# leoelm/Bayesian_inference_for_NN

Measured on NVIDIA B200. Metric: posterior_grad_evals_per_s, higher is better.
Workload: dtype f32 (tensor-core products on two int8 fixed-point slices per operand, kind::i8, exact int32 accumulate; f32 everywhere else)

## Files before the change

bayesian_inference_for_nn_b200/csrc/tc_fused.cuh:

```cuda
#pragma once
#include "tc_layer2.cuh"

namespace pyb {

constexpr int TF_THREADS = 384;
template <int CP> struct TfCfg {
  static constexpr int STAGES = 5;
  static constexpr int W2_BYTES = 2 * 256 * CP * 4;
  static constexpr int ZX_BYTES = 2 * CP * 128 * 4;
  static constexpr int SMEM = STAGES * TP_STAGE_BYTES + 1024  + 1024  + 2048  +
                              128  + W2_BYTES + ZX_BYTES;
  static constexpr int SMEM_I8 = SMEM + 4096;
};
__device__ __forceinline__ void tc_ld_16x256b_x4_raw(uint32_t taddr, uint32_t* r) {
  asm volatile(
      "tcgen05.ld.sync.aligned.16x256b.x4.b32 "
      "{%0, %1, %2, %3, %4, %5, %6, %7, %8, %9, %10, %11, %12, %13, %14, %15}, [%16];"
      : "=r"(r[0]), "=r"(r[1]), "=r"(r[2]), "=r"(r[3]), "=r"(r[4]), "=r"(r[5]), "=r"(r[6]), "=r"(r[7]), "=r"(r[8]),
        "=r"(r[9]), "=r"(r[10]), "=r"(r[11]), "=r"(r[12]), "=r"(r[13]), "=r"(r[14]), "=r"(r[15])
      : "r"(taddr)
      : "memory");
}
__device__ __forceinline__ void tc_mma_i8_pair(uint32_t tmem_d, uint64_t adesc, uint64_t bdesc, uint32_t idesc,
                                               uint32_t accumulate) {
  asm volatile(
      "{\n"
      ".reg .pred p;\n"
      "setp.ne.b32 p, %4, 0;\n"
      "tcgen05.mma.cta_group::2.kind::i8 [%0], %1, %2, %3, p;\n"
      "}\n" ::"r"(tmem_d),
      "l"(adesc), "l"(bdesc), "r"(idesc), "r"(accumulate)
      : "memory");
}
__device__ __forceinline__ void slice4_i8(const float* d, float zq, uint32_t& hw, uint32_t& lw) {
  constexpr float M = 12582912.0f;
  uint32_t hb[4], lb[4];
#pragma unroll
  for (int r = 0; r < 4; ++r) {
    const float t = fmaf(d[r], zq, M);
    const float h = t - M;
    const float e = fmaf(d[r], zq, -h);
    const float u = fmaf(e, 254.0f, M);
    hb[r] = __float_as_uint(t);
    lb[r] = __float_as_uint(u);
  }
  hw = __byte_perm(__byte_perm(hb[0], hb[1], 0x0040), __byte_perm(hb[2], hb[3], 0x0040), 0x5410);
  lw = __byte_perm(__byte_perm(lb[0], lb[1], 0x0040), __byte_perm(lb[2], lb[3], 0x0040), 0x5410);
}

__device__ __forceinline__ void tc_ld_16x256b_x4(uint32_t taddr, float* v) {
  uint32_t r[16];
  asm volatile(
      "tcgen05.ld.sync.aligned.16x256b.x4.b32 "
      "{%0, %1, %2, %3, %4, %5, %6, %7, %8, %9, %10, %11, %12, %13, %14, %15}, [%16];"
      : "=r"(r[0]), "=r"(r[1]), "=r"(r[2]), "=r"(r[3]), "=r"(r[4]), "=r"(r[5]), "=r"(r[6]), "=r"(r[7]), "=r"(r[8]),
        "=r"(r[9]), "=r"(r[10]), "=r"(r[11]), "=r"(r[12]), "=r"(r[13]), "=r"(r[14]), "=r"(r[15])
      : "r"(taddr)
      : "memory");
#pragma unroll
  for (int i = 0; i < 16; ++i) v[i] = __uint_as_float(r[i]);
}
template <int CP>
__device__ __forceinline__ int w2_slot(int h, int c) {
  return ((((h >> 3) * 2 + (h & 1)) * (CP / 4) + (c >> 2)) * 4 + ((h >> 1) & 3)) * 4 + (c & 3);
}
__device__ __forceinline__ void split_pair(float x0, float x1, uint32_t& hw, uint32_t& lw) {
  const __nv_bfloat162 hp = __floats2bfloat162_rn(x0, x1);
  hw = *reinterpret_cast<const uint32_t*>(&hp);
  const __nv_bfloat162 lp = __floats2bfloat162_rn(x0 - __uint_as_float(hw << 16), x1 - __uint_as_float(hw & 0xffff0000u));
  lw = *reinterpret_cast<const uint32_t*>(&lp);
}

template <int CP, bool FWD, int I8 = 0>
__global__ void __cluster_dims__(2, 1, 1) __launch_bounds__(TF_THREADS, 1)
tc_g1_layer2_fused(const __grid_constant__ CUtensorMap tmA_hi, const __grid_constant__ CUtensorMap tmA_lo,
                   const __grid_constant__ CUtensorMap tmB_hi, const __grid_constant__ CUtensorMap tmB_lo,
                   const TcGemmParams p, const Layer2Params l2) {
  constexpr int STAGES = TfCfg<CP>::STAGES;
  extern __shared__ uint8_t smem_raw[];
  uint8_t* smem = smem_raw + ((1024u - (smem_u32(smem_raw) & 1023u)) & 1023u);
  uint8_t* stage_base = smem;
  uint64_t* bars = (uint64_t*)(smem + STAGES * TP_STAGE_BYTES);
  uint64_t* full_bar = bars;
  uint64_t* empty_bar = bars + STAGES;
  uint64_t* tmem_full = bars + 2 * STAGES;
  uint64_t* tmem_empty = bars + 2 * STAGES + 2;
  uint32_t* tmem_ptr = (uint32_t*)(bars + 2 * STAGES + 4);
  float* bias_s = (float*)(smem + STAGES * TP_STAGE_BYTES + 1024);
  float* b2_s = bias_s + 512;
  float* W2_s = b2_s + 32;
  float* zx_s = W2_s + 2 * 256 * CP;
  float* cw_s = zx_s + 2 * CP * 128;
  float* zq_s = cw_s + 512;

  const int warp = __shfl_sync(0xffffffffu, (int)(threadIdx.x >> 5), 0), lane = threadIdx.x & 31;
  const uint32_t rank = cluster_ctarank();
  const int cluster_id = blockIdx.x >> 1, n_clusters = gridDim.x >> 1;
  constexpr int KSTAGE = I8 ? 64 : TC_BK;
  const int nk = (p.K + KSTAGE - 1) / KSTAGE;
  const int H = p.H;
  const int half_rows = H >> 1;
  const uint32_t cta_bytes = 2 * TC_A_TILE_BYTES + 2 * (uint32_t)half_rows * TC_BK * 2;

  if (warp == 8 && lane == 0) {
    asm volatile("prefetch.tensormap [%0];" ::"l"(&tmA_hi) : "memory");
    asm volatile("prefetch.tensormap [%0];" ::"l"(&tmA_lo) : "memory");
    asm volatile("prefetch.tensormap [%0];" ::"l"(&tmB_hi) : "memory");
    asm volatile("prefetch.tensormap [%0];" ::"l"(&tmB_lo) : "memory");
  }
  if (warp == 9 && lane == 0) {
    for (int s = 0; s < STAGES; ++s) { mbar_init(&full_bar[s], 1); mbar_init(&empty_bar[s], 1); }
    mbar_init(&tmem_full[0], 1); mbar_init(&tmem_full[1], 1);
    mbar_init(&tmem_empty[0], 16); mbar_init(&tmem_empty[1], 16);
    asm volatile("fence.mbarrier_init.release.cluster;" ::: "memory");
  }
  if (warp == 10) {
    asm volatile("tcgen05.alloc.cta_group::2.sync.aligned.shared::cta.b32 [%0], %1;" ::"r"(smem_u32(tmem_ptr)), "r"(512)
                 : "memory");
    asm volatile("tcgen05.relinquish_alloc_permit.cta_group::2.sync.aligned;" ::: "memory");
  }
  tc_fence_before();
  __syncthreads();
  cluster_sync_all();
  tc_fence_after();
  const uint32_t tmem_base = *tmem_ptr;

  if (warp >= 8) {
   asm volatile("setmaxnreg.dec.sync.aligned.u32 40;");
   if (warp == 8) {
    if (lane == 0) {
      int stage = 0;
      uint32_t phase = 0;
      for (int item = cluster_id; item < p.total_items; item += n_clusters) {
        int b, mp, split;
        tc_decode(p, item, b, mp, split);
        const int arow = p.a_row0 + (mp * 2 + (int)rank) * 128;
        const int brow = b * H + (int)rank * half_rows;
        for (int kc = 0; kc < nk; ++kc) {
          (I8 ? mbar_wait_sleep(&empty_bar[stage], phase ^ 1) : mbar_wait(&empty_bar[stage], phase ^ 1));
          uint8_t* st = stage_base + stage * TP_STAGE_BYTES;
          if (rank == 0) mbar_expect_tx(&full_bar[stage], 2 * cta_bytes);
          const int k0 = kc * KSTAGE;
          tma_load_2d_pair(st, &tmA_hi, &full_bar[stage], k0, arow);
          tma_load_2d_pair(st + TC_A_TILE_BYTES, &tmA_lo, &full_bar[stage], k0, arow);
          tma_load_2d_pair(st + 2 * TC_A_TILE_BYTES, &tmB_hi, &full_bar[stage], k0, brow);
          tma_load_2d_pair(st + 2 * TC_A_TILE_BYTES + 8192, &tmB_lo, &full_bar[stage], k0, brow);
          if (++stage == STAGES) { stage = 0; phase ^= 1; }
        }
      }
    }
  } else if (warp == 9) {
    if (rank == 0 && lane == 0) {
      const uint32_t idesc = (I8 ? (2u << 4) : (1u << 4)) | (1u << 7) | (1u << 10) | ((uint32_t)(H >> 3) << 17) | ((256u >> 4) << 24);
      int stage = 0, it = 0;
      uint32_t phase = 0;
      const int k_tail = p.K - (nk - 1) * KSTAGE;
      for (int item = cluster_id; item < p.total_items; item += n_clusters, ++it) {
        const int acc = I8 ? 0 : (it & 1);
        const uint32_t acc_phase = I8 ? (uint32_t)(it & 1) : (uint32_t)((it >> 1) & 1);
        (I8 ? mbar_wait_sleep(&tmem_empty[acc], acc_phase ^ 1) : mbar_wait(&tmem_empty[acc], acc_phase ^ 1));
        tc_fence_after();
        const uint32_t d = tmem_base + (uint32_t)acc * 256;
        for (int kc = 0; kc < nk; ++kc) {
          (I8 ? mbar_wait_sleep(&full_bar[stage], phase) : mbar_wait(&full_bar[stage], phase));
          tc_fence_after();
          const uint32_t st = smem_u32(stage_base + stage * TP_STAGE_BYTES);
          const int nks = (kc == nk - 1 && k_tail <= KSTAGE / 2) ? 1 : 2;
          for (int ks = 0; ks < nks; ++ks) {
            const uint32_t koff = ks * 32;
            const uint64_t ah = make_smem_desc_sw64(st + koff);
            const uint64_t al = make_smem_desc_sw64(st + TC_A_TILE_BYTES + koff);
            const uint64_t bh = make_smem_desc_sw64(st + 2 * TC_A_TILE_BYTES + koff);
            const uint64_t bl = make_smem_desc_sw64(st + 2 * TC_A_TILE_BYTES + 8192 + koff);
            const uint32_t accum = (kc != 0) || (ks != 0);
            if (I8) {
              tc_mma_i8_pair(d, ah, bh, idesc, accum);
              tc_mma_i8_pair(d + 256, ah, bl, idesc, accum);
              tc_mma_i8_pair(d + 256, al, bh, idesc, 1);
            } else {
              tc_mma_bf16_pair(d, ah, bh, idesc, accum);
              tc_mma_bf16_pair(d, al, bh, idesc, 1);
              tc_mma_bf16_pair(d, ah, bl, idesc, 1);
            }
          }
          tc_commit_pair(&empty_bar[stage]);
          if (++stage == STAGES) { stage = 0; phase ^= 1; }
        }
        tc_commit_pair(&tmem_full[acc]);
      }
    }
   }
  } else {
    asm volatile("setmaxnreg.inc.sync.aligned.u32 232;");
    const int half = warp >> 2;
    const int quad = warp & 3;
    const int g = lane >> 2, t = lane & 3;
    const int eall = threadIdx.x;
    const uint32_t lane_addr = (uint32_t)(quad * 32) << 16;
    const int Hh = H >> 1;
    const int C = l2.C;
    const float invN = l2.scale / (float)l2.N;
    const int r_own = 2 * (t & 1) + (t >> 1);
    const int row_own = quad * 32 + g + 8 * r_own;
    const int pos0 = quad * 32 + 4 * g;
    const int hbase = half * Hh + 2 * t;
    uint16_t* z2_hi = reinterpret_cast<uint16_t*>(l2.z2_hi);
    uint16_t* z2_lo = reinterpret_cast<uint16_t*>(l2.z2_lo);
    for (int i = eall; i < 2 * 256 * CP; i += 256) W2_s[i] = 0.f;
    if (eall < 32) b2_s[eall] = 0.f;
    asm volatile("bar.sync 1, 256;" ::: "memory");
    auto fetch_consts = [&](int item, int buf) {
      int b, mp, split;
      tc_decode(p, item, b, mp, split);
      const float* th = l2.theta + (int64_t)b * l2.P;
      if (eall < H) {
        const int h = eall;
        const float* src = th + l2.w2_off + (int64_t)h * C;
        const uint32_t dst = smem_u32(W2_s + buf * 256 * CP + w2_slot<CP>(h, 0));
#pragma unroll
        for (int c = 0; c < CP; ++c)
          if (c < C)
            asm volatile("cp.async.ca.shared.global [%0], [%1], 4;" ::"r"(dst + (uint32_t)(((c >> 2) * 16 + (c & 3)) * 4)),
                         "l"(src + c) : "memory");
        asm volatile("cp.async.ca.shared.global [%0], [%1], 4;" ::"r"(smem_u32(bias_s + buf * 256 + h)),
                     "l"(p.bias + (int64_t)b * p.bias_stride + h) : "memory");
      }
      if (eall < C)
        asm volatile("cp.async.ca.shared.global [%0], [%1], 4;" ::"r"(smem_u32(b2_s + buf * 16 + eall)),
                     "l"(th + l2.b2_off + eall) : "memory");
      if (I8 && eall < H) {
        asm volatile("cp.async.ca.shared.global [%0], [%1], 4;" ::"r"(smem_u32(cw_s + buf * 256 + eall)),
                     "l"(l2.cw + (int64_t)b * H + eall) : "memory");
        if (I8 == 2 && !FWD)
          asm volatile("cp.async.ca.shared.global [%0], [%1], 4;" ::"r"(smem_u32(zq_s + buf * 256 + eall)),
                       "l"(l2.zq + (int64_t)b * H + eall) : "memory");
      }
    };
    if (cluster_id < p.total_items) fetch_consts(cluster_id, 0);
    int it = 0;
    for (int item = cluster_id; item < p.total_items; item += n_clusters, ++it) {
      int b, mp, split;
      tc_decode(p, item, b, mp, split);
      const int mt = mp * 2 + (int)rank;
      const int cbuf = it & 1;
      const int acc = I8 ? 0 : cbuf;
      const uint32_t acc_phase = I8 ? (uint32_t)(it & 1) : (uint32_t)((it >> 1) & 1);
      float* bs = bias_s + cbuf * 256;
      float* b2b = b2_s + cbuf * 16;
      float* W2b = W2_s + cbuf * 256 * CP;
      float sxr[4] = {0.f, 0.f, 0.f, 0.f};
      if (I8) {
#pragma unroll
        for (int r = 0; r < 4; ++r) {
          const int rg = mt * 128 + quad * 32 + g + 8 * r;
          sxr[r] = rg < p.M_valid ? __ldg(l2.sx + rg) : 0.f;
        }
      }
      asm volatile("cp.async.wait_all;" ::: "memory");
      asm volatile("bar.sync 1, 256;" ::: "memory");
      (I8 ? mbar_wait_sleep(&tmem_full[acc], acc_phase) : mbar_wait(&tmem_full[acc], acc_phase));
      tc_fence_after();
      const int64_t blk_w = (((((int64_t)b * p.out_tiles + mt) * H) + hbase) * 128 + pos0) >> 2;
      uint2* pa_hi = reinterpret_cast<uint2*>(p.out_hi) + blk_w;
      uint2* pa_lo = reinterpret_cast<uint2*>(p.out_lo) + blk_w;
      uint2* pz_hi = reinterpret_cast<uint2*>(l2.zt_hi) + blk_w;
      uint2* pz_lo = reinterpret_cast<uint2*>(l2.zt_lo) + blk_w;
      const float4* w4b = reinterpret_cast<const float4*>(W2b) + (((half * Hh) >> 3) * 2 * (CP / 4)) * 4 + t;
      const float* bsb = bs + hbase;
      const float* cwb = cw_s + cbuf * 256 + hbase;
      const float* zqb = zq_s + cbuf * 256 + hbase;
      uint32_t* pzi_hi = nullptr; uint32_t* pzi_lo = nullptr;
      if (I8 == 2 && !FWD) {
        const int64_t blk_b = ((((int64_t)b * p.out_tiles + mt) * H) + hbase) * 128 + pos0;
        pzi_hi = reinterpret_cast<uint32_t*>(l2.zi_hi + blk_b);
        pzi_lo = reinterpret_cast<uint32_t*>(l2.zi_lo + blk_b);
      }
      float2 z[4][CP / 2];
#pragma unroll
      for (int r = 0; r < 4; ++r)
#pragma unroll
        for (int c = 0; c < CP / 2; ++c) z[r][c] = make_float2(0.f, 0.f);
      uint32_t mask[4] = {0u, 0u, 0u, 0u};
#pragma unroll
      for (int ch = 0; ch < 4; ++ch) {
        if (ch * 32 < Hh) {
          const uint32_t col = (uint32_t)(acc * 256 + half * Hh + ch * 32);
          float v[32];
          if (I8) {
#pragma unroll
            for (int hf = 0; hf < 2; ++hf) {
              uint32_t rh[16], rc[16];
              tc_ld_16x256b_x4_raw(tmem_base + lane_addr + ((uint32_t)(16 * hf) << 16) + col, rh);
              tc_ld_16x256b_x4_raw(tmem_base + lane_addr + ((uint32_t)(16 * hf) << 16) + 256u + col, rc);
              asm volatile("tcgen05.wait::ld.sync.aligned;" ::: "memory");
#pragma unroll
              for (int j = 0; j < 16; ++j)
                v[16 * hf + j] = fmaf((float)(int)rc[j], 1.0f / 254.0f, (float)(int)rh[j]);
            }
          } else {
            tc_ld_16x256b_x4(tmem_base + lane_addr + col, v);
            tc_ld_16x256b_x4(tmem_base + lane_addr + (16u << 16) + col, v + 16);
            asm volatile("tcgen05.wait::ld.sync.aligned;" ::: "memory");
          }
          uint32_t m = 0u;
#pragma unroll
          for (int kb = 0; kb < 4; ++kb) {
            const float2 bb = *reinterpret_cast<const float2*>(bsb + ch * 32 + 8 * kb);
            float2 cc = make_float2(0.f, 0.f);
            if (I8) cc = *reinterpret_cast<const float2*>(cwb + ch * 32 + 8 * kb);
            float a[4][2];
#pragma unroll
            for (int r = 0; r < 4; ++r) {
              const float* vv = v + (r >> 1) * 16 + kb * 4 + (r & 1) * 2;
              if (I8) {
                a[r][0] = fmaxf(fmaf(vv[0], sxr[r] * cc.x, bb.x), 0.f);
                a[r][1] = fmaxf(fmaf(vv[1], sxr[r] * cc.y, bb.y), 0.f);
              } else {
                a[r][0] = fmaxf(vv[0] + bb.x, 0.f);
                a[r][1] = fmaxf(vv[1] + bb.y, 0.f);
              }
              if (!FWD) {
                m |= (a[r][0] > 0.f ? 1u : 0u) << (kb * 8 + r * 2);
                m |= (a[r][1] > 0.f ? 1u : 0u) << (kb * 8 + r * 2 + 1);
              }
            }
#pragma unroll
            for (int i = 0; i < 2; ++i) {
              const float4* w4 = w4b + (((ch * 4 + kb) * 2 + i) * (CP / 4)) * 4;
#pragma unroll
              for (int c4 = 0; c4 < CP / 4; ++c4) {
                const float4 w = w4[c4 * 4];
                const float2 w01 = make_float2(w.x, w.y), w23 = make_float2(w.z, w.w);
#pragma unroll
                for (int r = 0; r < 4; ++r) {
                  const float2 aa = make_float2(a[r][i], a[r][i]);
                  z[r][2 * c4] = __ffma2_rn(aa, w01, z[r][2 * c4]);
                  z[r][2 * c4 + 1] = __ffma2_rn(aa, w23, z[r][2 * c4 + 1]);
                }
              }
              if (!FWD) {
                uint32_t hw0, lw0, hw1, lw1;
                split_pair(a[0][i], a[1][i], hw0, lw0);
                split_pair(a[2][i], a[3][i], hw1, lw1);
                const int w_off = (ch * 32 + 8 * kb + i) * 32;
                __stcs(pa_hi + w_off, make_uint2(hw0, hw1));
                __stcs(pa_lo + w_off, make_uint2(lw0, lw1));
              }
            }
          }
          mask[ch] = m;
        }
      }
      tc_fence_before();
      __syncwarp();
      if (lane == 0) mbar_arrive_leader_relaxed(&tmem_empty[acc]);
      if (item + n_clusters < p.total_items) fetch_consts(item + n_clusters, cbuf ^ 1);
      float zo[CP];
      {
        const bool b0 = t & 1, b1 = t & 2;
#pragma unroll
        for (int c = 0; c < CP; ++c) {
          const float z0 = (c & 1) ? z[0][c >> 1].y : z[0][c >> 1].x, z1 = (c & 1) ? z[1][c >> 1].y : z[1][c >> 1].x;
          const float z2v = (c & 1) ? z[2][c >> 1].y : z[2][c >> 1].x, z3 = (c & 1) ? z[3][c >> 1].y : z[3][c >> 1].x;
          float k0 = b0 ? z2v : z0, k1 = b0 ? z3 : z1;
          const float g0 = __shfl_xor_sync(0xffffffffu, b0 ? z0 : z2v, 1);
          const float g1 = __shfl_xor_sync(0xffffffffu, b0 ? z1 : z3, 1);
          k0 = b0 ? g0 + k0 : k0 + g0;
          k1 = b0 ? g1 + k1 : k1 + g1;
          const float kk = b1 ? k1 : k0;
          const float gg = __shfl_xor_sync(0xffffffffu, b1 ? k0 : k1, 2);
          zo[c] = b1 ? gg + kk : kk + gg;
        }
      }
#pragma unroll
      for (int c = 0; c < CP; ++c) zx_s[(half * CP + c) * 128 + row_own] = zo[c];
      asm volatile("bar.sync 2, 256;" ::: "memory");
      float zf[CP], dz[CP];
#pragma unroll
      for (int c = 0; c < CP; ++c) zf[c] = (b2b[c] + zx_s[c * 128 + row_own]) + zx_s[(CP + c) * 128 + row_own];
      const int row_g = mt * 128 + row_own;
      if (FWD) {
        if (half == 0 && row_g < p.M_valid) {
          float* o = l2.fwd_out + ((int64_t)b * l2.N + row_g) * C;
          if (l2.out_act == PYB_ACT_SOFTMAX) {
            float mx = -INFINITY;
#pragma unroll
            for (int c = 0; c < CP; ++c) if (c < C) mx = fmaxf(mx, zf[c]);
            float se = 0.f;
#pragma unroll
            for (int c = 0; c < CP; ++c) if (c < C) se += expf(zf[c] - mx);
            const float inv = 1.0f / se;
#pragma unroll
            for (int c = 0; c < CP; ++c) if (c < C) o[c] = expf(zf[c] - mx) * inv;
          } else {
#pragma unroll
            for (int c = 0; c < CP; ++c) if (c < C) o[c] = act_apply(zf[c], l2.out_act);
          }
        }
        continue;
      }
      float loss_r = 0.f;
      l2_loss_dz<CP>(l2, row_g, row_g < p.M_valid, zf, dz, loss_r, invN);
      if (half == 0) {
        const int64_t blk2 = (((int64_t)b * p.out_tiles + mt) * L2_CMAX) * 128 + pos0 + r_own;
#pragma unroll
        for (int c = 0; c < CP; ++c) {
          __nv_bfloat16 hb, lb;
          split_bf16(dz[c], hb, lb);
          z2_hi[blk2 + c * 128] = __bfloat16_as_ushort(hb);
          z2_lo[blk2 + c * 128] = __bfloat16_as_ushort(lb);
        }
        const int64_t grp = (int64_t)b * l2.n_groups + mt * 4 + quad;
        float mine = 0.f;
#pragma unroll
        for (int c = 0; c < CP; ++c) {
          const float sm = warp_sum(dz[c]);
          if (lane == c) mine = sm;
        }
        if (lane < CP) l2.b2_partial[grp * L2_CMAX + lane] = mine;
        const float ls = warp_sum(loss_r);
        if (lane == 0) l2.loss_partial[grp] = (double)ls;
      }
      float2 dzp[4][CP / 2];
#pragma unroll
      for (int r = 0; r < 4; ++r) {
        const int src = (lane & ~3) | ((r >> 1) | ((r & 1) << 1));
#pragma unroll
        for (int c = 0; c < CP / 2; ++c) {
          dzp[r][c].x = __shfl_sync(0xffffffffu, dz[2 * c], src);
          dzp[r][c].y = __shfl_sync(0xffffffffu, dz[2 * c + 1], src);
        }
      }
#pragma unroll
      for (int ch = 0; ch < 4; ++ch) {
        if (ch * 32 < Hh) {
          const uint32_t m = mask[ch];
#pragma unroll
          for (int kb = 0; kb < 4; ++kb) {
#pragma unroll
            for (int i = 0; i < 2; ++i) {
              const float4* w4 = w4b + (((ch * 4 + kb) * 2 + i) * (CP / 4)) * 4;
              float2 s[4];
#pragma unroll
              for (int r = 0; r < 4; ++r) s[r] = make_float2(0.f, 0.f);
#pragma unroll
              for (int c4 = 0; c4 < CP / 4; ++c4) {
                const float4 w = w4[c4 * 4];
                const float2 w01 = make_float2(w.x, w.y), w23 = make_float2(w.z, w.w);
#pragma unroll
                for (int r = 0; r < 4; ++r) {
                  s[r] = __ffma2_rn(dzp[r][2 * c4], w01, s[r]);
                  s[r] = __ffma2_rn(dzp[r][2 * c4 + 1], w23, s[r]);
                }
              }
              float d[4];
#pragma unroll
              for (int r = 0; r < 4; ++r) d[r] = ((m >> (kb * 8 + r * 2 + i)) & 1u) ? s[r].x + s[r].y : 0.f;
              const int w_off = (ch * 32 + 8 * kb + i) * 32;
              if (I8 == 2) {
                uint32_t hw, lw;
                slice4_i8(d, zqb[ch * 32 + 8 * kb + i], hw, lw);
                __stcs(pzi_hi + w_off, hw);
                __stcs(pzi_lo + w_off, lw);
              } else {
                uint32_t hw0, lw0, hw1, lw1;
                split_pair(d[0], d[1], hw0, lw0);
                split_pair(d[2], d[3], hw1, lw1);
                __stcs(pz_hi + w_off, make_uint2(hw0, hw1));
                __stcs(pz_lo + w_off, make_uint2(lw0, lw1));
              }
            }
          }
        }
      }
    }
  }
  tc_fence_before();
  __syncthreads();
  cluster_sync_all();
  if (warp == 10) {
    tc_fence_after();
    asm volatile("tcgen05.dealloc.cta_group::2.sync.aligned.b32 %0, %1;" ::"r"(tmem_base), "r"(512) : "memory");
  }
}

}
```

bayesian_inference_for_nn_b200/csrc/tc_path.cu:

```cuda
#include <cstdlib>
#include <cstring>
#include "tc_fused_mma.cuh"
#include <algorithm>

namespace pyb {

typedef CUresult (*PFN_encodeTiled)(CUtensorMap*, CUtensorMapDataType, cuuint32_t, void*, const cuuint64_t*,
                                    const cuuint64_t*, const cuuint32_t*, const cuuint32_t*, CUtensorMapInterleave,
                                    CUtensorMapSwizzle, CUtensorMapL2promotion, CUtensorMapFloatOOBfill);
static PFN_encodeTiled get_encode() {
  static PFN_encodeTiled fn = nullptr;
  if (!fn) {
    void* f = nullptr;
    cudaDriverEntryPointQueryResult q;
    PYB_CUDA(cudaGetDriverEntryPoint("cuTensorMapEncodeTiled", &f, cudaEnableDefault, &q));
    PYB_REQUIRE(f != nullptr && q == cudaDriverEntryPointSuccess, PYB_ERR_CUDA, "cuTensorMapEncodeTiled unavailable");
    fn = (PFN_encodeTiled)f;
  }
  return fn;
}
static CUtensorMap make_map_blocked(const void* base, int64_t blocks, int rows_per_block, int box_rows) {
  CUtensorMap m;
  cuuint64_t dims[3] = {128, (cuuint64_t)rows_per_block, (cuuint64_t)blocks};
  cuuint64_t strides[2] = {256, (cuuint64_t)rows_per_block * 256};
// ... 124 lines not shown
  tc_gemm_bf16x3<EPI, ACT><<<grid, TC_THREADS, TC_SMEM_BYTES, h->stream>>>(a_hi, a_lo, b_hi, b_lo, p);
}
template <int EPI, int ACT>
static void launch_pair_inst(pyb_handle* h, int grid, const CUtensorMap& a_hi, const CUtensorMap& a_lo,
                             const CUtensorMap& b_hi, const CUtensorMap& b_lo, const TcGemmParams& p) {
  PYB_CUDA(cudaFuncSetAttribute(tc_gemm_pair_bf16x3<EPI, ACT>, cudaFuncAttributeMaxDynamicSharedMemorySize, TP_SMEM_BYTES));
  tc_gemm_pair_bf16x3<EPI, ACT><<<grid, TP_THREADS, TP_SMEM_BYTES, h->stream>>>(a_hi, a_lo, b_hi, b_lo, p);
}
static bool pair_ok(const pyb_handle* h, const TcGemmParams& p) {
  if (!h->opt_tc_pair || p.b_blocked || p.H < 32 || p.n_mtiles < 2) return false;
  if (p.n_btiles > 0) return p.a_blocked && p.n_mtiles == 2 && (p.H % 16) == 0;
  if ((p.H % 32) != 0) return false;
  return !p.a_blocked && p.a_batch_rows == 0;
}
static void launch_gemm_tc(pyb_handle* h, const CUtensorMap& a_hi, const CUtensorMap& a_lo,
                           const CUtensorMap& b_hi, const CUtensorMap& b_lo, TcGemmParams p, double flops,
                           const CUtensorMap* bp_hi = nullptr, const CUtensorMap* bp_lo = nullptr) {
  if (p.k_splits <= 1) { p.k_splits = 1; p.chunks_per_split = (p.K + TC_BK - 1) / TC_BK; p.split_stride = 0; }
  p.vec_store = p.epi == EPI_STORE && ((uintptr_t)p.out % 16 == 0) && (p.out_stride % 4 == 0) && (p.out_ld % 4 == 0) &&
                (p.split_stride % 4 == 0);
  int grid = std::min(p.total_items, h->sm_count);
  prof_begin(h);
  if (bp_hi && bp_lo && pair_ok(h, p) && p.n_btiles > 1 && p.epi == EPI_STORE && p.transpose_out && h->opt_tc_dual &&
      p.H <= 256 && (p.H / 2) * TC_BK * 2 <= 8192) {
    p.total_items = p.n_batch * p.k_splits * ((p.n_btiles + 1) / 2);
    grid = std::min(2 * p.total_items, (h->sm_count / 2) * 2);
    PYB_CUDA(cudaFuncSetAttribute(tc_gemm_pair_dual_bf16x3, cudaFuncAttributeMaxDynamicSharedMemorySize, TD_SMEM_BYTES));
    tc_gemm_pair_dual_bf16x3<<<grid, TP_THREADS, TD_SMEM_BYTES, h->stream>>>(a_hi, a_lo, *bp_hi, *bp_lo, p);
    prof_end(h, flops);
    count_launch(h);
    return;
  }
  if (bp_hi && bp_lo && pair_ok(h, p)) {
    grid = std::min(2 * p.total_items, (h->sm_count / 2) * 2);
    if (p.epi == EPI_STORE) launch_pair_inst<EPI_STORE, 0>(h, grid, a_hi, a_lo, *bp_hi, *bp_lo, p);
    else if (p.act == PYB_ACT_RELU) launch_pair_inst<EPI_BIAS_ACT_T_SPLIT, PYB_ACT_RELU>(h, grid, a_hi, a_lo, *bp_hi, *bp_lo, p);
    else if (p.act == PYB_ACT_TANH) launch_pair_inst<EPI_BIAS_ACT_T_SPLIT, PYB_ACT_TANH>(h, grid, a_hi, a_lo, *bp_hi, *bp_lo, p);
    else if (p.act == PYB_ACT_SIGMOID) launch_pair_inst<EPI_BIAS_ACT_T_SPLIT, PYB_ACT_SIGMOID>(h, grid, a_hi, a_lo, *bp_hi, *bp_lo, p);
    else launch_pair_inst<EPI_BIAS_ACT_T_SPLIT, PYB_ACT_LINEAR>(h, grid, a_hi, a_lo, *bp_hi, *bp_lo, p);
    prof_end(h, flops);
    count_launch(h);
    return;
  }
  if (p.epi == EPI_STORE) launch_gemm_inst<EPI_STORE, 0>(h, grid, a_hi, a_lo, b_hi, b_lo, p);
  else if (p.act == PYB_ACT_RELU) launch_gemm_inst<EPI_BIAS_ACT_T_SPLIT, PYB_ACT_RELU>(h, grid, a_hi, a_lo, b_hi, b_lo, p);
  else if (p.act == PYB_ACT_TANH) launch_gemm_inst<EPI_BIAS_ACT_T_SPLIT, PYB_ACT_TANH>(h, grid, a_hi, a_lo, b_hi, b_lo, p);
  else if (p.act == PYB_ACT_SIGMOID) launch_gemm_inst<EPI_BIAS_ACT_T_SPLIT, PYB_ACT_SIGMOID>(h, grid, a_hi, a_lo, b_hi, b_lo, p);
  else launch_gemm_inst<EPI_BIAS_ACT_T_SPLIT, PYB_ACT_LINEAR>(h, grid, a_hi, a_lo, b_hi, b_lo, p);
  prof_end(h, flops);
  count_launch(h);
}


template <int CP, bool FWD, int I8>
static void launch_fused_i8(pyb_handle* h, int grid, const CUtensorMap& a_hi, const CUtensorMap& a_lo,
                            const CUtensorMap& b_hi, const CUtensorMap& b_lo, const TcGemmParams& p, const Layer2Params& l2) {
  PYB_CUDA(cudaFuncSetAttribute(tc_g1_layer2_fused<CP, FWD, I8>, cudaFuncAttributeMaxDynamicSharedMemorySize, TfCfg<CP>::SMEM_I8));
  tc_g1_layer2_fused<CP, FWD, I8><<<grid, TF_THREADS, TfCfg<CP>::SMEM_I8, h->stream>>>(a_hi, a_lo, b_hi, b_lo, p, l2);
}
template <int CP>
static void launch_fused_inst(pyb_handle* h, int grid, const CUtensorMap& a_hi, const CUtensorMap& a_lo,
                              const CUtensorMap& b_hi, const CUtensorMap& b_lo, const TcGemmParams& p, const Layer2Params& l2,
                              int i8 = 0) {
  if (i8 && !l2.fwd_out && h->opt_tc_epi_mma) {
    if (i8 >= 2) {
      PYB_CUDA(cudaFuncSetAttribute(tc_fused_i8_mma<CP, true>, cudaFuncAttributeMaxDynamicSharedMemorySize, TfmCfg::SMEM));
      tc_fused_i8_mma<CP, true><<<grid, TFM_THREADS, TfmCfg::SMEM, h->stream>>>(a_hi, a_lo, b_hi, b_lo, p, l2);
    } else {
      PYB_CUDA(cudaFuncSetAttribute(tc_fused_i8_mma<CP, false>, cudaFuncAttributeMaxDynamicSharedMemorySize, TfmCfg::SMEM));
      tc_fused_i8_mma<CP, false><<<grid, TFM_THREADS, TfmCfg::SMEM, h->stream>>>(a_hi, a_lo, b_hi, b_lo, p, l2);
    }
    return;
  }
  if (i8) {
    if (l2.fwd_out) launch_fused_i8<CP, true, 1>(h, grid, a_hi, a_lo, b_hi, b_lo, p, l2);
    else if (i8 >= 2) launch_fused_i8<CP, false, 2>(h, grid, a_hi, a_lo, b_hi, b_lo, p, l2);
    else launch_fused_i8<CP, false, 1>(h, grid, a_hi, a_lo, b_hi, b_lo, p, l2);
    return;
  }
  if (l2.fwd_out) {
    PYB_CUDA(cudaFuncSetAttribute(tc_g1_layer2_fused<CP, true>, cudaFuncAttributeMaxDynamicSharedMemorySize, TfCfg<CP>::SMEM));
    tc_g1_layer2_fused<CP, true><<<grid, TF_THREADS, TfCfg<CP>::SMEM, h->stream>>>(a_hi, a_lo, b_hi, b_lo, p, l2);
    return;
  }
  PYB_CUDA(cudaFuncSetAttribute(tc_g1_layer2_fused<CP, false>, cudaFuncAttributeMaxDynamicSharedMemorySize, TfCfg<CP>::SMEM));
  tc_g1_layer2_fused<CP, false><<<grid, TF_THREADS, TfCfg<CP>::SMEM, h->stream>>>(a_hi, a_lo, b_hi, b_lo, p, l2);
}
static bool fused_ok(const pyb_handle* h, int H, int act1) {
  return h->opt_tc_pair && h->opt_tc_fuse && act1 == PYB_ACT_RELU && (H == 128 || H == 256);
}

static int i8_mode(const pyb_handle* h, bool backward, bool resident) {
  const Model& m = h->model;
  int want = h->opt_tc_i8;
  if (want < 0) want = (resident && backward && h->i8_guard_ok) ? 2 : 0;
  if (want <= 0 || !fused_ok(h, m.layer[0].fan_out, m.layer[0].act) || m.layer[1].fan_out > L2_CMAX) return 0;
  if (m.layer[0].fan_in > 32768) return 0;
  if (!backward) return 1;
  const bool ce = h->loss_kind == PYB_LOSS_SPARSE_CE && m.layer[1].act == PYB_ACT_SOFTMAX;
  return (want >= 2 && ce && m.layer[0].fan_out == 256) ? 2 : 1;
}

static void tc_prepare_data_i8(pyb_handle* h, TcData& d, const float* X, int64_t N, int mode) {
  const int D = d.D;
  const int64_t Npad = d.Npad;
  d.Dk = (D + 15) / 16 * 16;
  d.col_mean.alloc(D); d.col_absmax.alloc(D); d.sx.alloc(N); d.sf.alloc(D + 1);
  d.xs_hi.alloc(N * d.Dk); d.xs_lo.alloc(N * d.Dk);
  d.stat_sum.alloc((size_t)I8_STAT_CHUNKS * D); d.stat_max.alloc((size_t)I8_STAT_CHUNKS * D);
  k_col_stats<<<dim3((D + 31) / 32, I8_STAT_CHUNKS), dim3(32, 32), 0, h->stream>>>(X, N, D, d.stat_sum.p, d.stat_max.p);
  k_col_stats_final<<<(D + 255) / 256, 256, 0, h->stream>>>(d.stat_sum.p, d.stat_max.p, I8_STAT_CHUNKS, N, D, d.col_mean.p,
                                                           d.col_absmax.p);
  count_launch(h);
  const int wpb = 8;
  k_slice_x_rows_i8<<<(unsigned)std::min<int64_t>((N + wpb - 1) / wpb, 8 * (int64_t)h->sm_count), wpb * 32, 0, h->stream>>>(
      X, N, D, d.col_mean.p, d.xs_hi.p, d.xs_lo.p, d.sx.p, d.Dk);
  count_launch(h, 2);
  d.mXs_hi = make_map_u8p(d.xs_hi.p, d.Dk, N, d.Dk, 128);
  d.mXs_lo = make_map_u8p(d.xs_lo.p, d.Dk, N, d.Dk, 128);
  if (mode >= 2) {
    d.xts_hi.alloc((int64_t)(D + 1) * Npad); d.xts_lo.alloc((int64_t)(D + 1) * Npad);
    PYB_CUDA(cudaMemsetAsync(d.xts_hi.p, 0, (size_t)(D + 1) * Npad, h->stream));
    PYB_CUDA(cudaMemsetAsync(d.xts_lo.p, 0, (size_t)(D + 1) * Npad, h->stream));
    dim3 g2((D + 31) / 32, (unsigned)((N + 31) / 32), 1), blk(32, 8);
    k_slice_xt_i8<<<g2, blk, 0, h->stream>>>(X, N, D, d.col_absmax.p, d.xts_hi.p, d.xts_lo.p, Npad);
    k_xt_i8_tail<<<(unsigned)((std::max<int64_t>(N, D + 1) + 255) / 256), 256, 0, h->stream>>>(
        d.xts_hi.p + (int64_t)D * Npad, N, d.col_absmax.p, d.sf.p, D);
    count_launch(h, 2);
// ... 89 lines not shown
    st->ws_hi.alloc(cc * H * Dk); st->ws_lo.alloc(cc * H * Dk);
    st->cw.alloc(cc * H); st->b1c.alloc(cc * H); st->zq.alloc(cc * H); st->zd.alloc(cc * H);
    st->mWs_hi = make_map_u8p(st->ws_hi.p, Dk, cc * H, Dk, H / 2);
    st->mWs_lo = make_map_u8p(st->ws_lo.p, Dk, cc * H, Dk, H / 2);
    if (mode >= 2) {
      st->cap_blocks_i8 = std::max(st->cap_blocks_i8, need_blocks);
      const int64_t cb = st->cap_blocks_i8;
      st->zi_hi.alloc(cb * H * 128); st->zi_lo.alloc(cb * H * 128);
      st->mZi_hi = make_map_blocked_u8(st->zi_hi.p, cb, H, 128);
      st->mZi_lo = make_map_blocked_u8(st->zi_lo.p, cb, H, 128);
    }
  }
  return bc;
}

static void tc_pack_and_g1(pyb_handle* h, TcState* st, TcData& d, const float* th, int nb,
                           const Layer2Params* fused = nullptr, int i8 = 0) {
  const Model& m = h->model;
  const LayerDesc& L1 = m.layer[0];
  const int D = st->D, H = st->H;
  const int64_t N = d.N, Npad = d.Npad, P = m.P;
  if (i8) {
    const float invN = fused->fwd_out ? 1.0f : fused->scale / (float)fused->N;
    k_pack_w1_i8<<<dim3((H + 31) / 32, nb), dim3(32, 8), 0, h->stream>>>(
        th, P, L1.w_off, L1.b_off, m.layer[1].w_off, D, H, m.layer[1].fan_out, d.col_mean.p, invN, st->ws_hi.p, st->ws_lo.p,
        d.Dk, st->cw.p, st->b1c.p, st->zq.p, st->zd.p);
  } else {
  dim3 g((H + 31) / 32, (D + 31) / 32, nb), blk(32, 8);
  k_split_transpose<<<g, blk, 0, h->stream>>>(th + L1.w_off, P, D, H, H, st->w_hi.p, st->w_lo.p, (int64_t)H * D, D);
  }
  count_launch(h);
  TcGemmParams p = {};
  p.K = D; p.n_mtiles = (int)(Npad / 128); p.n_pairs = (p.n_mtiles + 1) / 2; p.n_batch = nb; p.H = H;
  p.a_batch_rows = 0; p.a_box_rows = 128; p.order = 1; p.sub_batch = 32; p.total_items = p.n_pairs * nb;
  p.epi = EPI_BIAS_ACT_T_SPLIT;
  p.bias = th + L1.b_off; p.bias_stride = P; p.act = L1.act;
  p.out_hi = st->a_hi.p; p.out_lo = st->a_lo.p; p.out_tiles = (int)(Npad / 128);
  p.M_valid = (int)N; p.N_valid = H;
  if (fused) {
    const int grid = std::min(2 * p.total_items, (h->sm_count / 2) * 2);
    const int C = fused->C;
    Layer2Params f2 = *fused;
    const CUtensorMap &a_hi = i8 ? d.mXs_hi : d.mX_hi, &a_lo = i8 ? d.mXs_lo : d.mX_lo;
    const CUtensorMap &b_hi = i8 ? st->mWs_hi : st->mWp_hi, &b_lo = i8 ? st->mWs_lo : st->mWp_lo;
    if (i8) {
      p.bias = st->b1c.p; p.bias_stride = H;
      f2.dbg = nullptr; f2.dbg_flags = h->opt_tc_timeline & ~1;
      if (h->opt_tc_timeline) { st->dbg.alloc(8 * 160); f2.dbg = st->dbg.p; }
      f2.sx = d.sx.p; f2.cw = st->cw.p; f2.zq = st->zq.p; f2.zi_hi = st->zi_hi.p; f2.zi_lo = st->zi_lo.p;
    }
    prof_begin(h);
    if (C <= 4) launch_fused_inst<4>(h, grid, a_hi, a_lo, b_hi, b_lo, p, f2, i8);
    else if (C <= 8) launch_fused_inst<8>(h, grid, a_hi, a_lo, b_hi, b_lo, p, f2, i8);
    else if (C <= 12) launch_fused_inst<12>(h, grid, a_hi, a_lo, b_hi, b_lo, p, f2, i8);
    else launch_fused_inst<16>(h, grid, a_hi, a_lo, b_hi, b_lo, p, f2, i8);
    prof_end(h, 2.0 * N * (D * (double)H + (fused->fwd_out ? 1.0 : 3.0) * H * C) * nb);
    count_launch(h);
    return;
  }
  launch_gemm_tc(h, d.mX_hi, d.mX_lo, st->mW_hi, st->mW_lo, p, 2.0 * N * D * (double)H * nb, &st->mWp_hi, &st->mWp_lo);
}

static void tc_eval_on(pyb_handle* h, TcState* st, TcData& d, const int32_t* y_i, const float* y_f, const float* theta,
                       int64_t S, float scale, float* loss_out, float* grad_out) {
  const Model& m = h->model;
  const int64_t Bc = tc_prepare_bufs(h, st, S, d.Npad, true, d.i8);
  const LayerDesc& L1 = m.layer[0];
  const LayerDesc& L2 = m.layer[1];
  const int D = st->D, H = st->H, C = st->C;
  const int64_t N = d.N, Npad = d.Npad, P = m.P;
  const int n_tiles = (int)(Npad / L2_ROWS);
  const bool fused = fused_ok(h, H, L1.act) && C <= L2_CMAX;
  const int i8 = d.i8;
  const int n_groups = fused ? (int)(Npad / 128) * 4
                             : std::min(n_tiles, std::max(1, (int)((8 * (int64_t)h->sm_count + Bc - 1) / Bc)));
  st->b2_partial.alloc((size_t)Bc * n_groups * L2_CMAX);
  st->loss_partial.alloc((size_t)Bc * n_groups);
  for (int64_t b0 = 0; b0 < S; b0 += Bc) {
    const int nb = (int)std::min<int64_t>(Bc, S - b0);
    const float* th = theta + b0 * P;
    float* gr = grad_out + b0 * P;
    {
      Layer2Params p = {};
      p.a_hi = st->a_hi.p; p.a_lo = st->a_lo.p; p.zt_hi = st->z_hi.p; p.zt_lo = st->z_lo.p;
      p.z2_hi = st->z2_hi.p; p.z2_lo = st->z2_lo.p; p.k_tiles = (int)(Npad / 128);
      p.theta = th; p.P = P; p.w2_off = L2.w_off; p.b2_off = L2.b_off;
      p.H = H; p.C = C; p.N = (int)N; p.act1 = L1.act; p.out_act = L2.act; p.loss_kind = h->loss_kind;
      p.y_i = y_i; p.y_f = y_f; p.scale = scale;
      p.loss_partial = st->loss_partial.p; p.b2_partial = st->b2_partial.p; p.n_groups = n_groups;
      p.n_tiles = n_tiles;
      if (fused) {
        tc_pack_and_g1(h, st, d, th, nb, &p, i8);
      } else {
        tc_pack_and_g1(h, st, d, th, nb);
        dim3 g(n_groups, nb);
        if (C <= 4) k_layer2<4><<<g, 128, 0, h->stream>>>(p);
        else if (C <= 8) k_layer2<8><<<g, 128, 0, h->stream>>>(p);
        else if (C <= 12) k_layer2<12><<<g, 128, 0, h->stream>>>(p);
        else k_layer2<16><<<g, 128, 0, h->stream>>>(p);
      }
      k_layer2_reduce<<<nb, 256, 0, h->stream>>>(st->b2_partial.p, st->loss_partial.p, n_groups, C, gr, P, L2.b_off,
                                                loss_out ? loss_out + b0 : nullptr, (int)N);
      count_launch(h, 2);
    }
    const int nk_rows = (int)(Npad / TC_BK);
    const int splits = (nk_rows + TC_SPLIT_CHUNKS - 1) / TC_SPLIT_CHUNKS;
// ... 288 lines not shown
```

Before: 11340.

## Add CP=10 fused instance, prefetch TMEM chunks, split epilogue rows across halves

Adds a CP=10 specialization with a W2 shared-memory layout that packs a trailing pair of classes, so ten-class models do less padded work than under CP=12. The I8 epilogue now issues the TMEM loads for the next 32-column chunk before computing the current one, inlines the sparse cross-entropy loss/dz with the label prefetched early, and splits the per-row loss between the two warp halves with 64-thread named barriers instead of a 256-thread barrier. The dz values are exchanged through shared memory rather than warp shuffles. It also adds optional clock64 timeline instrumentation, enabled only when a debug buffer is present, and pads CP to a multiple of four for the MMA epilogue variant.

```diff
diff --git a/bayesian_inference_for_nn_b200/csrc/tc_fused.cuh b/bayesian_inference_for_nn_b200/csrc/tc_fused.cuh
--- a/bayesian_inference_for_nn_b200/csrc/tc_fused.cuh
+++ b/bayesian_inference_for_nn_b200/csrc/tc_fused.cuh
@@ -62,7 +62,8 @@
 }
 template <int CP>
 __device__ __forceinline__ int w2_slot(int h, int c) {
-  return ((((h >> 3) * 2 + (h & 1)) * (CP / 4) + (c >> 2)) * 4 + ((h >> 1) & 3)) * 4 + (c & 3);
+  const int seg = ((h >> 3) * 2 + (h & 1)) * 4 * CP, t = (h >> 1) & 3;
+  return c < CP / 4 * 4 ? seg + (c >> 2) * 16 + t * 4 + (c & 3) : seg + CP / 4 * 16 + t * 2 + (c & 1);
 }
 __device__ __forceinline__ void split_pair(float x0, float x1, uint32_t& hw, uint32_t& lw) {
   const __nv_bfloat162 hp = __floats2bfloat162_rn(x0, x1);
@@ -71,7 +72,7 @@
   lw = *reinterpret_cast<const uint32_t*>(&lp);
 }
 
-template <int CP, bool FWD, int I8 = 0>
+template <int CP, bool FWD, int I8 = 0, bool TL = false>
 __global__ void __cluster_dims__(2, 1, 1) __launch_bounds__(TF_THREADS, 1)
 tc_g1_layer2_fused(const __grid_constant__ CUtensorMap tmA_hi, const __grid_constant__ CUtensorMap tmA_lo,
                    const __grid_constant__ CUtensorMap tmB_hi, const __grid_constant__ CUtensorMap tmB_lo,
@@ -155,15 +156,20 @@
       int stage = 0, it = 0;
       uint32_t phase = 0;
       const int k_tail = p.K - (nk - 1) * KSTAGE;
+      long long t_wait = 0, t_loop = 0, t_fill = 0, c1 = 0;
       for (int item = cluster_id; item < p.total_items; item += n_clusters, ++it) {
         const int acc = I8 ? 0 : (it & 1);
         const uint32_t acc_phase = I8 ? (uint32_t)(it & 1) : (uint32_t)((it >> 1) & 1);
+        if (TL) c1 = clock64();
         (I8 ? mbar_wait_sleep(&tmem_empty[acc], acc_phase ^ 1) : mbar_wait(&tmem_empty[acc], acc_phase ^ 1));
         tc_fence_after();
+        if (TL) { const long long c = clock64(); t_wait += c - c1; c1 = c; }
         const uint32_t d = tmem_base + (uint32_t)acc * 256;
         for (int kc = 0; kc < nk; ++kc) {
+          const long long f0 = TL ? clock64() : 0;
           (I8 ? mbar_wait_sleep(&full_bar[stage], phase) : mbar_wait(&full_bar[stage], phase));
           tc_fence_after();
+          if (TL) t_fill += clock64() - f0;
           const uint32_t st = smem_u32(stage_base + stage * TP_STAGE_BYTES);
           const int nks = (kc == nk - 1 && k_tail <= KSTAGE / 2) ? 1 : 2;
           for (int ks = 0; ks < nks; ++ks) {
@@ -187,6 +193,13 @@
           if (++stage == STAGES) { stage = 0; phase ^= 1; }
         }
         tc_commit_pair(&tmem_full[acc]);
+        if (TL) t_loop += clock64() - c1;
+      }
+      if (TL) {
+        l2.dbg[blockIdx.x * 8 + 0] = (unsigned long long)t_wait;
+        l2.dbg[blockIdx.x * 8 + 1] = (unsigned long long)t_loop;
+        l2.dbg[blockIdx.x * 8 + 2] = (unsigned long long)t_fill;
+        l2.dbg[blockIdx.x * 8 + 3] = (unsigned long long)it;
       }
     }
    }
@@ -203,6 +216,9 @@
     const int r_own = 2 * (t & 1) + (t >> 1);
     const int row_own = quad * 32 + g + 8 * r_own;
     const int pos0 = quad * 32 + 4 * g;
+    const bool own_rows = half == (quad >> 1);
+    const bool ce = l2.loss_kind == PYB_LOSS_SPARSE_CE;
+    long long e_top = 0, e_wait = 0, e_A = 0, e_x = 0, e_sm = 0, e_B = 0;
     const int hbase = half * Hh + 2 * t;
     uint16_t* z2_hi = reinterpret_cast<uint16_t*>(l2.z2_hi);
     uint16_t* z2_lo = reinterpret_cast<uint16_t*>(l2.z2_lo);
@@ -220,7 +236,7 @@
 #pragma unroll
         for (int c = 0; c < CP; ++c)
           if (c < C)
-            asm volatile("cp.async.ca.shared.global [%0], [%1], 4;" ::"r"(dst + (uint32_t)(((c >> 2) * 16 + (c & 3)) * 4)),
+            asm volatile("cp.async.ca.shared.global [%0], [%1], 4;" ::"r"(dst + (uint32_t)((w2_slot<CP>(h, c) - w2_slot<CP>(h, 0)) * 4)),
                          "l"(src + c) : "memory");
         asm volatile("cp.async.ca.shared.global [%0], [%1], 4;" ::"r"(smem_u32(bias_s + buf * 256 + h)),
                      "l"(p.bias + (int64_t)b * p.bias_stride + h) : "memory");
@@ -239,9 +255,12 @@
     if (cluster_id < p.total_items) fetch_consts(cluster_id, 0);
     int it = 0;
     for (int item = cluster_id; item < p.total_items; item += n_clusters, ++it) {
+      const long long s0 = TL ? clock64() : 0;
       int b, mp, split;
       tc_decode(p, item, b, mp, split);
       const int mt = mp * 2 + (int)rank;
+      const int row_g = mt * 128 + row_own;
+      const int yi = (!FWD && ce && own_rows && row_g < p.M_valid) ? __ldg(l2.y_i + row_g) : 0;
       const int cbuf = it & 1;
       const int acc = I8 ? 0 : cbuf;
       const uint32_t acc_phase = I8 ? (uint32_t)(it & 1) : (uint32_t)((it >> 1) & 1);
@@ -258,14 +277,27 @@
       }
       asm volatile("cp.async.wait_all;" ::: "memory");
       asm volatile("bar.sync 1, 256;" ::: "memory");
+      const long long s1 = TL ? clock64() : 0;
       (I8 ? mbar_wait_sleep(&tmem_full[acc], acc_phase) : mbar_wait(&tmem_full[acc], acc_phase));
       tc_fence_after();
+      const long long s2 = TL ? clock64() : 0;
       const int64_t blk_w = (((((int64_t)b * p.out_tiles + mt) * H) + hbase) * 128 + pos0) >> 2;
       uint2* pa_hi = reinterpret_cast<uint2*>(p.out_hi) + blk_w;
       uint2* pa_lo = reinterpret_cast<uint2*>(p.out_lo) + blk_w;
       uint2* pz_hi = reinterpret_cast<uint2*>(l2.zt_hi) + blk_w;
       uint2* pz_lo = reinterpret_cast<uint2*>(l2.zt_lo) + blk_w;
-      const float4* w4b = reinterpret_cast<const float4*>(W2b) + (((half * Hh) >> 3) * 2 * (CP / 4)) * 4 + t;
+      const float* w2q = W2b + w2_slot<CP>(hbase, 0);
+      const float* w2d = W2b + w2_slot<CP>(hbase, CP - 1) - 1;
+      auto w2_row = [&](int ch, int kb, int i, float2* w) {
+        const int seg = ((ch * 4 + kb) * 2 + i) * 4 * CP;
+#pragma unroll
+        for (int c4 = 0; c4 < CP / 4; ++c4) {
+          const float4 v = *reinterpret_cast<const float4*>(w2q + seg + c4 * 16);
+          w[2 * c4] = make_float2(v.x, v.y);
+          w[2 * c4 + 1] = make_float2(v.z, v.w);
+        }
+        if (CP % 4) w[CP / 2 - 1] = *reinterpret_cast<const float2*>(w2d + seg);
+      };
       const float* bsb = bs + hbase;
       const float* cwb = cw_s + cbuf * 256 + hbase;
       const float* zqb = zq_s + cbuf * 256 + hbase;
@@ -281,22 +313,29 @@
 #pragma unroll
         for (int c = 0; c < CP / 2; ++c) z[r][c] = make_float2(0.f, 0.f);
       uint32_t mask[4] = {0u, 0u, 0u, 0u};
+      uint32_t rh[2][16], rc[2][16];
+      auto ld_chunk = [&](int ch) {
+        const uint32_t col = (uint32_t)(half * Hh + ch * 32);
+#pragma unroll
+        for (int hf = 0; hf < 2; ++hf) {
+          tc_ld_16x256b_x4_raw(tmem_base + lane_addr + ((uint32_t)(16 * hf) << 16) + col, rh[hf]);
+          tc_ld_16x256b_x4_raw(tmem_base + lane_addr + ((uint32_t)(16 * hf) << 16) + 256u + col, rc[hf]);
+        }
+      };
+      if (I8) ld_chunk(0);
 #pragma unroll
       for (int ch = 0; ch < 4; ++ch) {
         if (ch * 32 < Hh) {
           const uint32_t col = (uint32_t)(acc * 256 + half * Hh + ch * 32);
           float v[32];
           if (I8) {
-#pragma unroll
-            for (int hf = 0; hf < 2; ++hf) {
-              uint32_t rh[16], rc[16];
-              tc_ld_16x256b_x4_raw(tmem_base + lane_addr + ((uint32_t)(16 * hf) << 16) + col, rh);
-              tc_ld_16x256b_x4_raw(tmem_base + lane_addr + ((uint32_t)(16 * hf) << 16) + 256u + col, rc);
-              asm volatile("tcgen05.wait::ld.sync.aligned;" ::: "memory");
+            asm volatile("tcgen05.wait::ld.sync.aligned;" ::: "memory");
+#pragma unroll
+            for (int hf = 0; hf < 2; ++hf)
 #pragma unroll
               for (int j = 0; j < 16; ++j)
-                v[16 * hf + j] = fmaf((float)(int)rc[j], 1.0f / 254.0f, (float)(int)rh[j]);
-            }
+                v[16 * hf + j] = fmaf((float)(int)rc[hf][j], 1.0f / 254.0f, (float)(int)rh[hf][j]);
+            if ((ch + 1) * 32 < Hh) ld_chunk(ch + 1);
           } else {
             tc_ld_16x256b_x4(tmem_base + lane_addr + col, v);
             tc_ld_16x256b_x4(tmem_base + lane_addr + (16u << 16) + col, v + 16);
@@ -326,18 +365,12 @@
             }
 #pragma unroll
             for (int i = 0; i < 2; ++i) {
-              const float4* w4 = w4b + (((ch * 4 + kb) * 2 + i) * (CP / 4)) * 4;
-#pragma unroll
-              for (int c4 = 0; c4 < CP / 4; ++c4) {
-                const float4 w = w4[c4 * 4];
-                const float2 w01 = make_float2(w.x, w.y), w23 = make_float2(w.z, w.w);
-#pragma unroll
-                for (int r = 0; r < 4; ++r) {
-                  const float2 aa = make_float2(a[r][i], a[r][i]);
-                  z[r][2 * c4] = __ffma2_rn(aa, w01, z[r][2 * c4]);
-                  z[r][2 * c4 + 1] = __ffma2_rn(aa, w23, z[r][2 * c4 + 1]);
-                }
-              }
+              float2 w[CP / 2];
+              w2_row(ch, kb, i, w);
+#pragma unroll
+              for (int c2 = 0; c2 < CP / 2; ++c2)
+#pragma unroll
+                for (int r = 0; r < 4; ++r) z[r][c2] = __ffma2_rn(make_float2(a[r][i], a[r][i]), w[c2], z[r][c2]);
               if (!FWD) {
                 uint32_t hw0, lw0, hw1, lw1;
                 split_pair(a[0][i], a[1][i], hw0, lw0);
@@ -354,6 +387,7 @@
       tc_fence_before();
       __syncwarp();
       if (lane == 0) mbar_arrive_leader_relaxed(&tmem_empty[acc]);
+      const long long s3 = TL ? clock64() : 0;
       if (item + n_clusters < p.total_items) fetch_consts(item + n_clusters, cbuf ^ 1);
       float zo[CP];
       {
@@ -374,34 +408,55 @@
       }
 #pragma unroll
       for (int c = 0; c < CP; ++c) zx_s[(half * CP + c) * 128 + row_own] = zo[c];
-      asm volatile("bar.sync 2, 256;" ::: "memory");
-      float zf[CP], dz[CP];
-#pragma unroll
-      for (int c = 0; c < CP; ++c) zf[c] = (b2b[c] + zx_s[c * 128 + row_own]) + zx_s[(CP + c) * 128 + row_own];
-      const int row_g = mt * 128 + row_own;
-      if (FWD) {
-        if (half == 0 && row_g < p.M_valid) {
-          float* o = l2.fwd_out + ((int64_t)b * l2.N + row_g) * C;
-          if (l2.out_act == PYB_ACT_SOFTMAX) {
+      asm volatile("bar.sync %0, 64;" ::"r"(3 + quad) : "memory");
+      const long long s4 = TL ? clock64() : 0;
+      if (own_rows) {
+        float zf[CP], dz[CP];
+#pragma unroll
+        for (int c = 0; c < CP; ++c) zf[c] = (b2b[c] + zx_s[c * 128 + row_own]) + zx_s[(CP + c) * 128 + row_own];
+        if (FWD) {
+          if (row_g < p.M_valid) {
+            float* o = l2.fwd_out + ((int64_t)b * l2.N + row_g) * C;
+            if (l2.out_act == PYB_ACT_SOFTMAX) {
+              float mx = -INFINITY;
+#pragma unroll
+              for (int c = 0; c < CP; ++c) if (c < C) mx = fmaxf(mx, zf[c]);
+              float se = 0.f;
+#pragma unroll
+              for (int c = 0; c < CP; ++c) if (c < C) se += expf(zf[c] - mx);
+              const float inv = 1.0f / se;
+#pragma unroll
+              for (int c = 0; c < CP; ++c) if (c < C) o[c] = expf(zf[c] - mx) * inv;
+            } else {
+#pragma unroll
+              for (int c = 0; c < CP; ++c) if (c < C) o[c] = act_apply(zf[c], l2.out_act);
+            }
+          }
+          continue;
+        }
+        float loss_r = 0.f;
+        if (ce) {
+#pragma unroll
+          for (int c = 0; c < CP; ++c) dz[c] = 0.f;
+          if (row_g < p.M_valid) {
             float mx = -INFINITY;
 #pragma unroll
             for (int c = 0; c < CP; ++c) if (c < C) mx = fmaxf(mx, zf[c]);
             float se = 0.f;
 #pragma unroll
-            for (int c = 0; c < CP; ++c) if (c < C) se += expf(zf[c] - mx);
+            for (int c = 0; c < CP; ++c) if (c < C) { dz[c] = expf(zf[c] - mx); se += dz[c]; }
+            float zy = 0.f;
+#pragma unroll
+            for (int c = 0; c < CP; ++c) if (c == yi) zy = zf[c];
+            loss_r += logf(se) - (zy - mx);
             const float inv = 1.0f / se;
 #pragma unroll
-            for (int c = 0; c < CP; ++c) if (c < C) o[c] = expf(zf[c] - mx) * inv;
-          } else {
-#pragma unroll
-            for (int c = 0; c < CP; ++c) if (c < C) o[c] = act_apply(zf[c], l2.out_act);
+            for (int c = 0; c < CP; ++c)
+              if (c < C) dz[c] = (dz[c] * inv - (c == yi ? 1.f : 0.f)) * invN;
           }
-        }
-        continue;
-      }
-      float loss_r = 0.f;
-      l2_loss_dz<CP>(l2, row_g, row_g < p.M_valid, zf, dz, loss_r, invN);
-      if (half == 0) {
+        } else {
+          l2_loss_dz<CP>(l2, row_g, row_g < p.M_valid, zf, dz, loss_r, invN);
+        }
         const int64_t blk2 = (((int64_t)b * p.out_tiles + mt) * L2_CMAX) * 128 + pos0 + r_own;
 #pragma unroll
         for (int c = 0; c < CP; ++c) {
@@ -420,17 +475,20 @@
         if (lane < CP) l2.b2_partial[grp * L2_CMAX + lane] = mine;
         const float ls = warp_sum(loss_r);
         if (lane == 0) l2.loss_partial[grp] = (double)ls;
-      }
-      float2 dzp[4][CP / 2];
-#pragma unroll
-      for (int r = 0; r < 4; ++r) {
-        const int src = (lane & ~3) | ((r >> 1) | ((r & 1) << 1));
-#pragma unroll
-        for (int c = 0; c < CP / 2; ++c) {
-          dzp[r][c].x = __shfl_sync(0xffffffffu, dz[2 * c], src);
-          dzp[r][c].y = __shfl_sync(0xffffffffu, dz[2 * c + 1], src);
-        }
-      }
+        __syncwarp();
+#pragma unroll
+        for (int c = 0; c < CP; ++c) zx_s[c * 128 + pos0 + r_own] = dz[c];
+      }
+      if (FWD) continue;
+      asm volatile("bar.sync %0, 64;" ::"r"(3 + quad) : "memory");
+      float2 dzp[CP][2];
+#pragma unroll
+      for (int c = 0; c < CP; ++c) {
+        const float4 d4 = *reinterpret_cast<const float4*>(zx_s + c * 128 + pos0);
+        dzp[c][0] = make_float2(d4.x, d4.y);
+        dzp[c][1] = make_float2(d4.z, d4.w);
+      }
+      const long long s5 = TL ? clock64() : 0;
 #pragma unroll
       for (int ch = 0; ch < 4; ++ch) {
         if (ch * 32 < Hh) {
@@ -439,23 +497,22 @@
           for (int kb = 0; kb < 4; ++kb) {
 #pragma unroll
             for (int i = 0; i < 2; ++i) {
-              const float4* w4 = w4b + (((ch * 4 + kb) * 2 + i) * (CP / 4)) * 4;
-              float2 s[4];
-#pragma unroll
-              for (int r = 0; r < 4; ++r) s[r] = make_float2(0.f, 0.f);
-#pragma unroll
-              for (int c4 = 0; c4 < CP / 4; ++c4) {
-                const float4 w = w4[c4 * 4];
-                const float2 w01 = make_float2(w.x, w.y), w23 = make_float2(w.z, w.w);
-#pragma unroll
-                for (int r = 0; r < 4; ++r) {
-                  s[r] = __ffma2_rn(dzp[r][2 * c4], w01, s[r]);
-                  s[r] = __ffma2_rn(dzp[r][2 * c4 + 1], w23, s[r]);
-                }
+              float2 w[CP / 2];
+              w2_row(ch, kb, i, w);
+              float2 s[2][2];
+#pragma unroll
+              for (int e = 0; e < 2; ++e) s[e][0] = s[e][1] = make_float2(0.f, 0.f);
+#pragma unroll
+              for (int c = 0; c < CP; ++c) {
+                const float wc = (c & 1) ? w[c >> 1].y : w[c >> 1].x;
+#pragma unroll
+                for (int rp = 0; rp < 2; ++rp) s[c & 1][rp] = __ffma2_rn(dzp[c][rp], make_float2(wc, wc), s[c & 1][rp]);
               }
+              const float se[4] = {s[0][0].x, s[0][0].y, s[0][1].x, s[0][1].y};
+              const float so[4] = {s[1][0].x, s[1][0].y, s[1][1].x, s[1][1].y};
               float d[4];
 #pragma unroll
-              for (int r = 0; r < 4; ++r) d[r] = ((m >> (kb * 8 + r * 2 + i)) & 1u) ? s[r].x + s[r].y : 0.f;
+              for (int r = 0; r < 4; ++r) d[r] = ((m >> (kb * 8 + r * 2 + i)) & 1u) ? se[r] + so[r] : 0.f;
               const int w_off = (ch * 32 + 8 * kb + i) * 32;
               if (I8 == 2) {
                 uint32_t hw, lw;
@@ -473,6 +530,17 @@
           }
         }
       }
+      if (TL) { e_top += s1 - s0; e_wait += s2 - s1; e_A += s3 - s2; e_x += s4 - s3; e_sm += s5 - s4; e_B += clock64() - s5; }
+    }
+    if (TL && warp == 0 && lane == 0) {
+      if (blockIdx.x & 1) {
+        l2.dbg[blockIdx.x * 8 + 0] = (unsigned long long)e_x;
+        l2.dbg[blockIdx.x * 8 + 1] = (unsigned long long)e_sm;
+      }
+      l2.dbg[blockIdx.x * 8 + 4] = (unsigned long long)e_top;
+      l2.dbg[blockIdx.x * 8 + 5] = (unsigned long long)e_wait;
+      l2.dbg[blockIdx.x * 8 + 6] = (unsigned long long)e_A;
+      l2.dbg[blockIdx.x * 8 + 7] = (unsigned long long)e_B;
     }
   }
   tc_fence_before();
diff --git a/bayesian_inference_for_nn_b200/csrc/tc_path.cu b/bayesian_inference_for_nn_b200/csrc/tc_path.cu
--- a/bayesian_inference_for_nn_b200/csrc/tc_path.cu
+++ b/bayesian_inference_for_nn_b200/csrc/tc_path.cu
@@ -200,28 +200,30 @@
 }
 
 
-template <int CP, bool FWD, int I8>
+template <int CP, bool FWD, int I8, bool TL = false>
 static void launch_fused_i8(pyb_handle* h, int grid, const CUtensorMap& a_hi, const CUtensorMap& a_lo,
                             const CUtensorMap& b_hi, const CUtensorMap& b_lo, const TcGemmParams& p, const Layer2Params& l2) {
-  PYB_CUDA(cudaFuncSetAttribute(tc_g1_layer2_fused<CP, FWD, I8>, cudaFuncAttributeMaxDynamicSharedMemorySize, TfCfg<CP>::SMEM_I8));
-  tc_g1_layer2_fused<CP, FWD, I8><<<grid, TF_THREADS, TfCfg<CP>::SMEM_I8, h->stream>>>(a_hi, a_lo, b_hi, b_lo, p, l2);
+  PYB_CUDA(cudaFuncSetAttribute(tc_g1_layer2_fused<CP, FWD, I8, TL>, cudaFuncAttributeMaxDynamicSharedMemorySize, TfCfg<CP>::SMEM_I8));
+  tc_g1_layer2_fused<CP, FWD, I8, TL><<<grid, TF_THREADS, TfCfg<CP>::SMEM_I8, h->stream>>>(a_hi, a_lo, b_hi, b_lo, p, l2);
 }
 template <int CP>
 static void launch_fused_inst(pyb_handle* h, int grid, const CUtensorMap& a_hi, const CUtensorMap& a_lo,
                               const CUtensorMap& b_hi, const CUtensorMap& b_lo, const TcGemmParams& p, const Layer2Params& l2,
                               int i8 = 0) {
   if (i8 && !l2.fwd_out && h->opt_tc_epi_mma) {
+    constexpr int CPM = (CP + 3) / 4 * 4;
     if (i8 >= 2) {
-      PYB_CUDA(cudaFuncSetAttribute(tc_fused_i8_mma<CP, true>, cudaFuncAttributeMaxDynamicSharedMemorySize, TfmCfg::SMEM));
-      tc_fused_i8_mma<CP, true><<<grid, TFM_THREADS, TfmCfg::SMEM, h->stream>>>(a_hi, a_lo, b_hi, b_lo, p, l2);
+      PYB_CUDA(cudaFuncSetAttribute(tc_fused_i8_mma<CPM, true>, cudaFuncAttributeMaxDynamicSharedMemorySize, TfmCfg::SMEM));
+      tc_fused_i8_mma<CPM, true><<<grid, TFM_THREADS, TfmCfg::SMEM, h->stream>>>(a_hi, a_lo, b_hi, b_lo, p, l2);
     } else {
-      PYB_CUDA(cudaFuncSetAttribute(tc_fused_i8_mma<CP, false>, cudaFuncAttributeMaxDynamicSharedMemorySize, TfmCfg::SMEM));
-      tc_fused_i8_mma<CP, false><<<grid, TFM_THREADS, TfmCfg::SMEM, h->stream>>>(a_hi, a_lo, b_hi, b_lo, p, l2);
+      PYB_CUDA(cudaFuncSetAttribute(tc_fused_i8_mma<CPM, false>, cudaFuncAttributeMaxDynamicSharedMemorySize, TfmCfg::SMEM));
+      tc_fused_i8_mma<CPM, false><<<grid, TFM_THREADS, TfmCfg::SMEM, h->stream>>>(a_hi, a_lo, b_hi, b_lo, p, l2);
     }
     return;
   }
   if (i8) {
     if (l2.fwd_out) launch_fused_i8<CP, true, 1>(h, grid, a_hi, a_lo, b_hi, b_lo, p, l2);
+    else if (i8 >= 2 && l2.dbg) launch_fused_i8<CP, false, 2, true>(h, grid, a_hi, a_lo, b_hi, b_lo, p, l2);
     else if (i8 >= 2) launch_fused_i8<CP, false, 2>(h, grid, a_hi, a_lo, b_hi, b_lo, p, l2);
     else launch_fused_i8<CP, false, 1>(h, grid, a_hi, a_lo, b_hi, b_lo, p, l2);
     return;
@@ -417,6 +419,7 @@
     prof_begin(h);
     if (C <= 4) launch_fused_inst<4>(h, grid, a_hi, a_lo, b_hi, b_lo, p, f2, i8);
     else if (C <= 8) launch_fused_inst<8>(h, grid, a_hi, a_lo, b_hi, b_lo, p, f2, i8);
+    else if (C <= 10) launch_fused_inst<10>(h, grid, a_hi, a_lo, b_hi, b_lo, p, f2, i8);
     else if (C <= 12) launch_fused_inst<12>(h, grid, a_hi, a_lo, b_hi, b_lo, p, f2, i8);
     else launch_fused_inst<16>(h, grid, a_hi, a_lo, b_hi, b_lo, p, f2, i8);
     prof_end(h, 2.0 * N * (D * (double)H + (fused->fwd_out ? 1.0 : 3.0) * H * C) * nb);
```

After: 11460, median of 6. +1.1%, better.
